# trevordblack/Physically_Based_Renderer

Measured on AMD Instinct MI355X. Metric: shaded pixels/sec (Mpix/s) + achieved HBM GB/s, 4K G-buffer, 64 lights, higher is better.
Workload: dtype f32

## Files before the change

physically_based_renderer_amd/csrc/pbr_balanced.h:

```cpp
#pragma once
#include <cstdint>
#include <type_traits>

#include "pbr_device_math.h"
#include "pbr_device_math_x2.h"
#include "shade_kernels.h"

namespace pbr {

constexpr int kBalRec = 7;

#ifndef PBR_BAL_PROFILE
#define PBR_BAL_PROFILE 0
#endif
#if PBR_BAL_PROFILE
static __device__ unsigned long long* g_bal_prof_buf;
#define BAL_PROF_T(v) const long long v = (long long)__builtin_amdgcn_s_memtime()
#define BAL_PROF_ADD(slot_, val_) do { if ((threadIdx.x & 63) == 0) bal_prof[slot_] += (unsigned long long)(val_); } while (0)
#else
#define BAL_PROF_T(v)
#define BAL_PROF_ADD(i, x)
#endif

constexpr int kBalLdsStride = kBalMaxLights + 4;
// ... 185 lines not shown
}

__device__ __forceinline__ void wave_lds_sync() {
    __builtin_amdgcn_fence(__ATOMIC_RELEASE, "wavefront");
    __builtin_amdgcn_wave_barrier();
    __builtin_amdgcn_fence(__ATOMIC_ACQUIRE, "wavefront");
}
__device__ __forceinline__ void group_lds_sync(bool block) {
    if (block) {
        asm volatile("s_waitcnt lgkmcnt(0)" ::: "memory");
        __syncthreads();
    } else {
        wave_lds_sync();
    }
}

template <bool FINITE>
__device__ __forceinline__ float bal_wave_min(float v) {
    if constexpr (FINITE) return wave_min_finite(v);
    else return wave_min_dpp(v);
}
template <bool FINITE>
__device__ __forceinline__ float bal_wave_max(float v) {
    if constexpr (FINITE) return wave_max_finite(v);
    else return wave_max_dpp(v);
}
template <bool FINITE>
__device__ __forceinline__ float bal_fmin(float a, float b) {
    if constexpr (FINITE) return fmin_finite(a, b);
    else return fminf(a, b);
}
template <bool FINITE>
__device__ __forceinline__ float bal_fmax(float a, float b) {
    if constexpr (FINITE) return fmax_finite(a, b);
    else return fmaxf(a, b);
}

__device__ __forceinline__ void push_skip_bits4(uint32_t& ma, uint32_t& mb, float4 x, float4 y, float4 z,
                                                const f3x2& n, v2 kb) {
    const v2 x01 = v2{x.x, x.y}, x23 = v2{x.z, x.w}, y01 = v2{y.x, y.y}, y23 = v2{y.z, y.w};
    const v2 z01 = v2{z.x, z.y}, z23 = v2{z.z, z.w};
    const v2 ta01 = vfma(splat(n.x.x), x01, vfma(splat(n.y.x), y01, vfma(splat(n.z.x), z01, splat(kb.x))));
    const v2 ta23 = vfma(splat(n.x.x), x23, vfma(splat(n.y.x), y23, vfma(splat(n.z.x), z23, splat(kb.x))));
    const v2 tb01 = vfma(splat(n.x.y), x01, vfma(splat(n.y.y), y01, vfma(splat(n.z.y), z01, splat(kb.y))));
    const v2 tb23 = vfma(splat(n.x.y), x23, vfma(splat(n.y.y), y23, vfma(splat(n.z.y), z23, splat(kb.y))));
    ma = __builtin_amdgcn_alignbit(ma, __float_as_uint(ta23.y), 31);
    mb = __builtin_amdgcn_alignbit(mb, __float_as_uint(tb23.y), 31);
    ma = __builtin_amdgcn_alignbit(ma, __float_as_uint(ta23.x), 31);
    mb = __builtin_amdgcn_alignbit(mb, __float_as_uint(tb23.x), 31);
    ma = __builtin_amdgcn_alignbit(ma, __float_as_uint(ta01.y), 31);
    mb = __builtin_amdgcn_alignbit(mb, __float_as_uint(tb01.y), 31);
    ma = __builtin_amdgcn_alignbit(ma, __float_as_uint(ta01.x), 31);
    mb = __builtin_amdgcn_alignbit(mb, __float_as_uint(tb01.x), 31);
}

__device__ __forceinline__ void read_pair_lights(const float* lds_lights, int j0, int j1, f3x2& lp, f3x2& ls) {
    typedef __attribute__((address_space(3))) const float lds_float;
    j0 = PBR_BOUNDS(j0, kBalMaxLights + 1, kBoundsLds);
    j1 = PBR_BOUNDS(j1, kBalMaxLights + 1, kBoundsLds);
    const uint32_t base = (uint32_t)(uintptr_t)(const lds_float*)lds_lights;
    const uint32_t a0 = base + 4u * (uint32_t)j0, a1 = base + 4u * (uint32_t)j1;
    float x0, x1, y0, y1, z0, z1, r0, r1, g0, g1, u0, u1;
    static_assert(kBalLdsStride * 4 == 272, "offsets below");
    asm volatile(
        "ds_read_b32 %0, %12\n\t"
        "ds_read_b32 %1, %13\n\t"
        "ds_read_b32 %2, %12 offset:272\n\t"
        "ds_read_b32 %3, %13 offset:272\n\t"
        "ds_read_b32 %4, %12 offset:544\n\t"
        "ds_read_b32 %5, %13 offset:544\n\t"
        "ds_read_b32 %6, %12 offset:816\n\t"
        "ds_read_b32 %7, %13 offset:816\n\t"
        "ds_read_b32 %8, %12 offset:1088\n\t"
        "ds_read_b32 %9, %13 offset:1088\n\t"
        "ds_read_b32 %10, %12 offset:1360\n\t"
        "ds_read_b32 %11, %13 offset:1360\n\t"
        "s_waitcnt lgkmcnt(0)"
        : "=&v"(x0), "=&v"(x1), "=&v"(y0), "=&v"(y1), "=&v"(z0), "=&v"(z1), "=&v"(r0), "=&v"(r1), "=&v"(g0),
          "=&v"(g1), "=&v"(u0), "=&v"(u1)
        : "v"(a0), "v"(a1)
        : "memory");
    lp = f3x2{v2{x0, x1}, v2{y0, y1}, v2{z0, z1}};
    ls = f3x2{v2{r0, r1}, v2{g0, g1}, v2{u0, u1}};
}

constexpr float kBalNearVL = 0.0625f;
static_assert(PBR_POW5_FAST3_GLIBC_FROM >= 1.0f - 0.5f * kBalNearVL + 0x1p-14f,
              "a |V + L| >= kBalNearVL item has x < 0.9688: pow5_fast3's glibc band (a build switch) must start above it");
__device__ __forceinline__ void faithful_point_items2(const ItemPixel& q, const f3x2& lp, const f3x2& ls, m2& ok,
                                                      f3x2& sum, uint64_t live) {
    f3x2 l = f3x2{lp.x - q.pos.x, lp.y - q.pos.y, lp.z - q.pos.z};
    const v2 dist = sqrt_nr(dot3(l, l));
    const Recip2 rdist = recip_nr(dist);
    l = f3x2{div_nr(l.x, rdist), div_nr(l.y, rdist), div_nr(l.z, rdist)};
    const f3x2 vl = f3x2{q.v.x + l.x, q.v.y + l.y, q.v.z + l.z};
    const v2 svl = sqrt_nr(dot3(vl, vl));
    const Recip2 rvl = recip_nr(svl);
    const f3x2 h = f3x2{div_nr(vl.x, rvl), div_nr(vl.y, rvl), div_nr(vl.z, rvl)};
    const v2 att = rdist.r * rdist.r;
    const f3x2 n = splat3(q.n.x, q.n.y, q.n.z);
    const v2 n_dot_h = dot3_sat(n, h);
    const v2 inner = ((n_dot_h * n_dot_h) * q.a2m1 + 1.0f);
    const v2 den = inner * inner;
    const v2 n_dot_l = dot3_sat(n, l);
    const v2 r = rcp_hw((den * vfma(n_dot_l, splat(q.omk), splat(q.k))) * vfma(splat(q.nv), n_dot_l, splat(0.001f)));
    const v2 x = 1.0f - dot3_sat(h, splat3(q.v.x, q.v.y, q.v.z));
// ... 6 lines not shown
        if (x.y > PBR_POW5_FAST3_GLIBC_FROM && on(live)) p.y = pow5_glibc(x.y);
    }
    const f3x2 f = f3x2{q.f0.x + q.omf0.x * p, q.f0.y + q.omf0.y * p, q.f0.z + q.omf0.z * p};
    const v2 kr = (q.a2gv * n_dot_l) * r;
    const v2 w = att * n_dot_l;
    sum.x = vfma(vfma(kr, f.x, vfma(-f.x, splat(q.mab.x), splat(q.mab.x))), ls.x * w, sum.x);
    sum.y = vfma(vfma(kr, f.y, vfma(-f.y, splat(q.mab.y), splat(q.mab.y))), ls.y * w, sum.y);
    sum.z = vfma(vfma(kr, f.z, vfma(-f.z, splat(q.mab.z), splat(q.mab.z))), ls.z * w, sum.z);
}

__device__ __forceinline__ f3x2 exact_point_items2(const ItemPixelX& p, const f3x2& lp, const f3x2& ls, m2& ok,
                                                   uint64_t live) {
    PixelInvariants2 q;
    q.n = splat3(p.n.x, p.n.y, p.n.z);
    q.v = splat3(p.v.x, p.v.y, p.v.z);
    q.albedo = splat3(p.albedo.x, p.albedo.y, p.albedo.z);
    q.f0 = splat3(p.f0.x, p.f0.y, p.f0.z);
    q.one_minus_f0 = splat3(p.omf0.x, p.omf0.y, p.omf0.z);
    q.one_minus_metal = splat(p.omm);
    q.a_sqr = splat(p.a_sqr);
    q.a_sqr_minus_1 = splat(p.a2m1);
    q.k = splat(p.k);
    q.one_minus_k = splat(p.omk);
    q.ggx_v = splat(p.ggx_v);
    q.four_n_dot_v = splat(p.nv4);
    q.f0_nonzero = m2{~0ull, ~0ull};
    f3x2 l = f3x2{lp.x - p.pos.x, lp.y - p.pos.y, lp.z - p.pos.z};
    const v2 dist = sqrt_nr(dot3(l, l));
    const Recip2 rdist = recip_nr(dist);
    l = f3x2{div_nr(l.x, rdist), div_nr(l.y, rdist), div_nr(l.z, rdist)};
    const f3x2 h = normalize_x2(add3(q.v, l), ok);
    const v2 dsat = max_dsat(dist);
    const v2 att = recip_nr(dsat * dsat).r;
    return brdf_x2<true, true>(q, f3x2{ls.x * att, ls.y * att, ls.z * att}, l, h, ok, live);
}

struct BalMasks {
    uint32_t a0, a1, c0, c1;
    bool near_a, near_b;
};

constexpr float kBalDistLoFaithful = 0.01f;
constexpr float kBalDistLoExact = 0x1p-20f;

__device__ __forceinline__ m2 beyond_range(const f3x2& pos, float lx, float ly, float lz) {
    const f3x2 l = f3x2{splat(lx) - pos.x, splat(ly) - pos.y, splat(lz) - pos.z};
    const v2 x = dot3(l, l);
    return mask2(x.x > 10000.0f, x.y > 10000.0f);
}

template <bool EXACT>
__device__ __forceinline__ BalMasks balanced_pass1(const f3x2& pos, const f3x2& n, bool live_a, bool live_b, int nl,
                                                   float dist_lo, BalancedWaveLds& w, const float* lds_lights,
                                                   unsigned long long* bal_prof = nullptr) {
    const int lane_id = (int)(threadIdx.x & 63);
    BAL_PROF_T(t0);
    const float big = 3.0e38f;
    const f3 pa = lane(pos, 0), pb = lane(pos, 1);
    constexpr bool F = !EXACT;
    const float mnx = bal_wave_min<F>(bal_fmin<F>(live_a ? pa.x : big, live_b ? pb.x : big));
    const float mny = bal_wave_min<F>(bal_fmin<F>(live_a ? pa.y : big, live_b ? pb.y : big));
    const float mnz = bal_wave_min<F>(bal_fmin<F>(live_a ? pa.z : big, live_b ? pb.z : big));
    const float mxx = bal_wave_max<F>(bal_fmax<F>(live_a ? pa.x : -big, live_b ? pb.x : -big));
    const float mxy = bal_wave_max<F>(bal_fmax<F>(live_a ? pa.y : -big, live_b ? pb.y : -big));
    const float mxz = bal_wave_max<F>(bal_fmax<F>(live_a ? pa.z : -big, live_b ? pb.z : -big));
    const float cx = 0.5f * mnx + 0.5f * mxx, cy = 0.5f * mny + 0.5f * mxy, cz = 0.5f * mnz + 0.5f * mxz;
    const float r = (0.5f * (mxx - mnx) + 0.5f * (mxy - mny)) + 0.5f * (mxz - mnz);
    const float slack = r + (fabsf(cx) + fabsf(cy) + fabsf(cz)) * 0x1p-22f;
    const float pmax = bal_wave_max<F>(bal_fmax<F>(live_a ? (fabsf(pa.x) + fabsf(pa.y)) + fabsf(pa.z) : 0.0f,
                                                   live_b ? (fabsf(pb.x) + fabsf(pb.y)) + fabsf(pb.z) : 0.0f));
    float bj = 0.0f;
    bool near = true, far = false;
    bool close = false;
    if (lane_id < nl) {
        const float lx = lds_lights[lane_id], ly = lds_lights[kBalLdsStride + lane_id],
                    lz = lds_lights[2 * kBalLdsStride + lane_id];
        const float b0 = ((fabsf(lx - cx) + fabsf(ly - cy)) + fabsf(lz - cz)) + slack;
        const float fr = ((fabsf(lx) + fabsf(ly)) + fabsf(lz)) + pmax;
        bj = (b0 + 0.125f * fr) * (1.0f + 0x1p-20f);
        const float fx = fmaxf(fabsf(lx - mnx), fabsf(lx - mxx)), fy = fmaxf(fabsf(ly - mny), fabsf(ly - mxy)),
                    fz = fmaxf(fabsf(lz - mnz), fabsf(lz - mxz));
        const float gx = fmaxf(fmaxf(mnx - lx, lx - mxx), 0.0f), gy = fmaxf(fmaxf(mny - ly, ly - mxy), 0.0f),
                    gz = fmaxf(fmaxf(mnz - lz, lz - mxz), 0.0f);
        near = (fx * fx + fy * fy) + fz * fz <= 99.9f * 99.9f;
        far = (gx * gx + gy * gy) + gz * gz >= 100.1f * 100.1f;
        close = !((gx * gx + gy * gy) + gz * gz >= (1.02f * dist_lo) * (1.02f * dist_lo));
    }
    const float bmax = bal_wave_max<F>(bj);
    const uint64_t far_m = lanes(far), cross_m = lanes(!near && !far), close_m = lanes(close);
    const v2 cn = v2{0x1p-18f * ((fabsf(n.x.x) + fabsf(n.y.x)) + fabsf(n.z.x)),
                     0x1p-18f * ((fabsf(n.x.y) + fabsf(n.y.y)) + fabsf(n.z.y))};
    const v2 nd = -vfma(n.z, pos.z, vfma(n.y, pos.y, n.x * pos.x));
    const v2 kb = vfma(cn, splat(bmax), nd);
    uint32_t a0 = 0, a1 = 0, c0 = 0, c1 = 0;
    typedef __attribute__((address_space(3))) const float lds_float;
    const uint32_t lbase = (uint32_t)(uintptr_t)(const lds_float*)lds_lights;
    auto word = [&](int qbase, uint32_t& ma, uint32_t& mb) {
        for (int k = 6; k >= 0; k -= 2) {
            const uint32_t la = lbase + 16u * (uint32_t)(qbase + k);
            float4 x1, y1, z1, x0, y0, z0;
            asm volatile(
                "ds_read_b128 %0, %6 offset:16\n\t"
                "ds_read_b128 %1, %6 offset:288\n\t"
                "ds_read_b128 %2, %6 offset:560\n\t"
                "ds_read_b128 %3, %6\n\t"
                "ds_read_b128 %4, %6 offset:272\n\t"
                "ds_read_b128 %5, %6 offset:544\n\t"
                "s_waitcnt lgkmcnt(0)"
                : "=&v"(x1), "=&v"(y1), "=&v"(z1), "=&v"(x0), "=&v"(y0), "=&v"(z0)
                : "v"(la)
                : "memory");
            push_skip_bits4(ma, mb, x1, y1, z1, n, kb);
            push_skip_bits4(ma, mb, x0, y0, z0, n, kb);
        }
    };
    const int n0 = nl < 32 ? nl : 32;
    if (nl > 32) word(8, a1, c1);
    word(0, a0, c0);
    const int n1 = nl - n0;
    const uint32_t k0 = (n0 == 32 ? ~0u : (1u << n0) - 1u) & ~(uint32_t)far_m,
                   k1 = (n1 == 32 ? ~0u : (1u << n1) - 1u) & ~(uint32_t)(far_m >> 32);
    a0 = live_a ? ~a0 & k0 : 0u;
    c0 = live_b ? ~c0 & k0 : 0u;
    a1 = live_a ? ~a1 & k1 : 0u;
    c1 = live_b ? ~c1 & k1 : 0u;
    for (uint64_t cm = cross_m; cm != 0; cm &= cm - 1) {
        const int j = __builtin_ctzll(cm);
        const m2 out = beyond_range(pos, lds_lights[j], lds_lights[kBalLdsStride + j], lds_lights[2 * kBalLdsStride + j]);
        const uint32_t bit = 1u << (j & 31);
        const uint32_t oa = on(out.x) ? bit : 0u, ob = on(out.y) ? bit : 0u;
        if (j < 32) {
            a0 &= ~oa;
            c0 &= ~ob;
        } else {
            a1 &= ~oa;
            c1 &= ~ob;
        }
    }
    bool near_a = false, near_b = false;
    for (uint64_t cm = close_m; cm != 0; cm &= cm - 1) {
        const int j = __builtin_ctzll(cm);
        const f3x2 l = f3x2{splat(lds_lights[j]) - pos.x, splat(lds_lights[kBalLdsStride + j]) - pos.y,
                            splat(lds_lights[2 * kBalLdsStride + j]) - pos.z};
        const m2 ok = ge(sqrt_nr(dot3(l, l)), dist_lo);
        const uint32_t bit = 1u << (j & 31);
        near_a = near_a || (((j < 32 ? a0 : a1) & bit) != 0 && !on(ok.x));
        near_b = near_b || (((j < 32 ? c0 : c1) & bit) != 0 && !on(ok.y));
    }

    BAL_PROF_T(t1);
    BAL_PROF_ADD(0, t1 - t0);
    return BalMasks{a0, a1, c0, c1, near_a, near_b};
}

__device__ __forceinline__ int wave_live_items(const BalMasks& bm) {
    return wave_sum_dpp((__popc(bm.a0) + __popc(bm.a1)) + (__popc(bm.c0) + __popc(bm.c1)));
}


template <bool EXACT>
__device__ __forceinline__ void lighting_balanced_points(const PixelInvariants2& q, const Faithful2& fi,
                                                         const f3x2& pos, bool live_a, bool live_b, BalMasks bm,
                                                         BalancedWaveLds& w, const float* lds_lights, f3x2& sum,
                                                         m2& redo, unsigned long long* bal_prof = nullptr) {
    const int lane_id = (int)(threadIdx.x & 63);
    const uint32_t a0 = bm.a0, a1 = bm.a1, c0 = bm.c0, c1 = bm.c1;
    redo |= mask2(bm.near_a, bm.near_b);
    constexpr int R = EXACT ? kBalRecX : kBalRec;
    BAL_PROF_T(t1);
    PBR_PHASE("rank");

// ... 154 lines not shown
```

physically_based_renderer_amd/csrc/pbr_census.h:

```cpp
#pragma once

#ifndef PBR_CENSUS
#define PBR_CENSUS 0
#endif
#if PBR_CENSUS
#define PBR_PHASE(name)                          \
    do {                                         \
        __builtin_amdgcn_sched_barrier(0);       \
        asm volatile("; @phase " name);          \
        __builtin_amdgcn_sched_barrier(0);       \
    } while (0)
#else
#define PBR_PHASE(name) \
    do {                \
    } while (0)
#endif
#define PBR_COLD(name) PBR_PHASE("cold_" name)
```

physically_based_renderer_amd/csrc/pbr_context.hip:

```cpp
#include <cmath>
#include <cstdlib>
#include <cstring>
#include <new>

#include "pbr_context_impl.h"
#include "pbr_debug_bounds.h"
#include "pbr_build_info.h"

extern "C" {
extern const char pbr_unit_info_shade_kernels[] __attribute__((weak));
extern const char pbr_unit_info_shade_kernels_bal[] __attribute__((weak));
extern const char pbr_unit_info_frontend_kernels[] __attribute__((weak));
extern const char pbr_unit_info_pbr_frontend[] __attribute__((weak));
extern const char pbr_unit_info_gbuffer_fill[] __attribute__((weak));
__attribute__((used)) const char pbr_unit_info_pbr_context[] =
    PBR_UNIT_INFO("pbr_context", PBR_BI_SWITCH(PBR_DEBUG_BOUNDS));
}

namespace {

constexpr float kQuarterStrengthLo = 0x1p-34f, kQuarterStrengthHi = 0x1p50f;

constexpr float kFaithfulStrengthLo = 0x1p-25f, kFaithfulStrengthHi = 0x1p50f;

// ... 139 lines not shown
    return PBR_OK;
}

extern "C" {

int pbr_abi_version(void) { return PBR_ABI_VERSION; }

const char* pbr_build_info(void) {
    static const std::string info = [] {
        std::string r = "{\"abi\": " + std::to_string(PBR_ABI_VERSION) + ", \"units\": [";
        bool first = true;
        for (const char* u : {pbr_unit_info_pbr_context, pbr_unit_info_pbr_frontend, pbr_unit_info_shade_kernels,
                              pbr_unit_info_shade_kernels_bal, pbr_unit_info_frontend_kernels,
                              pbr_unit_info_gbuffer_fill}) {
            if (u == nullptr) continue;
            r += first ? "" : ", ";
            r += u;
            first = false;
        }
        return r + "]}";
    }();
    return info.c_str();
}

const char* pbr_strerror(int status) {
    switch (status) {
        case PBR_OK: return "ok";
        case PBR_ERR_INVALID_ARGUMENT: return "invalid argument";
        case PBR_ERR_NO_DEVICE: return "no HIP device";
        case PBR_ERR_OUT_OF_MEMORY: return "out of device memory";
        case PBR_ERR_LAUNCH: return "kernel launch failed";
        case PBR_ERR_HIP: return "HIP runtime error";
        case PBR_ERR_NOT_READY: return "pass or environment map not set";
        case PBR_ERR_UNSUPPORTED: return "unsupported";
        default: return "unknown status";
    }
}

const char* pbr_last_error(const pbr_context* ctx) { return ctx ? ctx->last_error.c_str() : ""; }

int pbr_context_create(int device, pbr_context** out_ctx) {
    if (!out_ctx) return PBR_ERR_INVALID_ARGUMENT;
    *out_ctx = nullptr;
    int count = 0;
    if (hipGetDeviceCount(&count) != hipSuccess || count <= 0) return PBR_ERR_NO_DEVICE;
    if (device < 0 || device >= count) return PBR_ERR_INVALID_ARGUMENT;
    pbr_context* ctx = new (std::nothrow) pbr_context();
    if (!ctx) return PBR_ERR_OUT_OF_MEMORY;
    ctx->device = device;
    if (const char* e = std::getenv("PBR_PIXELS_PER_THREAD")) ctx->pixels_per_thread = std::atoi(e) == 1 ? 1 : 2;
    if (const char* e = std::getenv("PBR_BALANCED_MIN")) ctx->balanced_min = std::atoi(e);
    if (const char* e = std::getenv("PBR_LEAN")) ctx->lean = std::atoi(e) != 0;
    if (const char* e = std::getenv("PBR_RANK_PER_WAVE")) ctx->rank_per_wave = std::atoi(e) != 0;
    DeviceGuard g(device);
    if (!g.ok) {
        delete ctx;
        return PBR_ERR_NO_DEVICE;
    }
    hipError_t e = arm_bounds(device);
    for (int i = 0; e == hipSuccess && i < pbr_context::kSlots; ++i) {
        e = hipHostMalloc(reinterpret_cast<void**>(&ctx->slots[i].h), sizeof(pbr_light) * PBR_MAX_LIGHTS,
                          hipHostMallocDefault);
        if (e == hipSuccess) e = hipEventCreateWithFlags(&ctx->slots[i].copied, hipEventDisableTiming);
    }
    if (e != hipSuccess) {
        pbr_context_destroy(ctx);
        return e == hipErrorOutOfMemory ? PBR_ERR_OUT_OF_MEMORY : PBR_ERR_HIP;
    }
    *out_ctx = ctx;
    return PBR_OK;
}

int pbr_context_destroy(pbr_context* ctx) {
    if (!ctx) return PBR_ERR_INVALID_ARGUMENT;
    {
        DeviceGuard g(ctx->device);
        (void)hipDeviceSynchronize();
        for (Resource* r : ctx->resources) {
            for (void** m : r->mem)
                if (m && *m) (void)hipFreeAsync(*m, nullptr);
            if (r->written) (void)hipEventDestroy(r->written);
        }
        for (pbr_context::LightSlot& sl : ctx->slots) {
            if (sl.copied) (void)hipEventDestroy(sl.copied);
            if (sl.h) (void)hipHostFree(sl.h);
        }
        for (StreamState& st : ctx->streams) release_stream_state(st);
        (void)hipDeviceSynchronize();
    }
    delete ctx;
    return PBR_OK;
}

int pbr_set_pass(pbr_context* ctx, const pbr_pass_desc* pass, void* stream) {
    if (!ctx || !pass) return PBR_ERR_INVALID_ARGUMENT;
    const int nd = pass->num_dir_lights, np = pass->num_point_lights, ns = pass->num_spot_lights;
    if (nd < 0 || np < 0 || ns < 0) return PBR_ERR_INVALID_ARGUMENT;
    const long long n = (long long)nd + np + ns;
    if (n > PBR_MAX_LIGHTS) return PBR_ERR_INVALID_ARGUMENT;
    if (n > 0 && !pass->lights) return PBR_ERR_INVALID_ARGUMENT;
    if (!is_ambient_mode(pass->ambient_mode)) return PBR_ERR_INVALID_ARGUMENT;
    const uint32_t known =
        PBR_FLAG_F0_PLANE | PBR_FLAG_APPLY_AO | PBR_FLAG_TILED_CULLING | PBR_FLAG_EXACT_ONLY | PBR_FLAG_FAITHFUL |
        PBR_FLAG_ALPHA_TEST;
    if (pass->flags & ~known) return PBR_ERR_INVALID_ARGUMENT;

// ... 146 lines not shown
    const bool alpha_test = (ctx->flags & PBR_FLAG_ALPHA_TEST) != 0;
    if (alpha_test && !gb->opacity) return PBR_ERR_INVALID_ARGUMENT;
    if (ctx->ambient_mode == PBR_AMBIENT_IBL_DIFFUSE && !ctx->env.d) return PBR_ERR_NOT_READY;
    if (fr->coverage && !ctx->sky.d) return PBR_ERR_NOT_READY;

    pbr::LaunchArgs a{};
    const float* planes[15] = {gb->pos_w[0], gb->pos_w[1], gb->pos_w[2], gb->normal_w[0], gb->normal_w[1],
                               gb->normal_w[2], gb->albedo[0], gb->albedo[1], gb->albedo[2], gb->metallic,
                               gb->roughness, gb->ao, gb->f0[0], gb->f0[1], gb->f0[2]};
    for (int i = 0; i < 15; ++i) a.gb.plane[i] = planes[i] ? planes[i] : planes[0];
    a.gb.plane[15] = alpha_test ? gb->opacity : planes[0];
    a.gb.alpha_test = alpha_test;
    a.gb.width = gb->width;
    a.gb.height = gb->height;
    a.gb.row_stride = gb->row_stride;
    a.gb.pairs_aligned = (gb->row_stride % 2) == 0;
    for (int i = 0; i < 16; ++i)
        if (!aligned(a.gb.plane[i], 8)) a.gb.pairs_aligned = false;
    a.ps = ctx->pass;
    a.ps.env_w = ctx->env.w;
    a.ps.env_h = ctx->env.h;
    a.ps.sky_w = ctx->sky.w;
    a.ps.sky_h = ctx->sky.h;
    a.lights = ctx->cur_slot >= 0 ? ctx->slots[ctx->cur_slot].d : nullptr;
    a.env = ctx->env.d;
    a.frame.out = fr->out;
    a.frame.out_stride = fr->out_row_stride;
    a.frame.format = fr->format == PBR_OUTPUT_RGBA8_UNORM ? pbr::kOutRgba8 : pbr::kOutRgba32f;
    a.frame.coverage = fr->coverage;
    a.frame.coverage_stride = fr->coverage_row_stride;
    a.frame.sky = ctx->sky.d;
    a.frame.width = gb->width - (debug_bounds_skew() ? 1 : 0);
    a.frame.height = gb->height;
    a.ambient_mode = ctx->ambient_mode;
    a.f0_plane = f0_plane;
    a.apply_ao = apply_ao;
    a.cull = cull;
    a.exact_only = (ctx->flags & PBR_FLAG_EXACT_ONLY) != 0;
    a.ps.faithful = (ctx->flags & PBR_FLAG_FAITHFUL) && !a.exact_only && ctx->faithful_pass_ok &&
                    (ctx->ambient_mode != PBR_AMBIENT_IBL_DIFFUSE || ctx->env.faithful_ok);
    if (a.ps.faithful && ctx->faithful_count_terms) a.ps.faithful = 2;
    a.pixels_per_thread = ctx->pixels_per_thread;
    constexpr int kBalancedMinFaithful = 22, kBalancedMinExact = 18;
    const int bal_min = ctx->balanced_min >= 0 ? ctx->balanced_min
                        : a.ps.faithful == 1   ? kBalancedMinFaithful
                                               : kBalancedMinExact;
    const bool bal_ok = !cull && a.pixels_per_thread == 2 && bal_min > 0 && ctx->points_flag_ok &&
                        a.ps.n_spot == 0 && a.ps.n_point >= bal_min && a.ps.n_point <= pbr::kBalMaxLights;
    a.ps.balanced = !bal_ok                                                ? 0
                    : a.ps.faithful == 1                                   ? 1
                    : a.ps.faithful == 0 && !a.exact_only && a.ps.n_dir == 0 && ctx->points_quarter_ok ? 2
                                                                           : 0;
    if (a.ps.balanced != 0 && ctx->rank_per_wave) a.ps.balanced |= pbr::kBalRankPerWave;

    if (const int rc = en.open(stream, "shade stream")) return rc;
    const hipStream_t s = en.s;
    const int si = en.si;
    hipError_t e = hipSuccess;
    StreamState& st = ctx->streams[si];
    {
        const int64_t tiles = pbr::shade_tile_count(gb->width, gb->height, a.pixels_per_thread);
        const int64_t slots = tiles * pbr::shade_stat_slots_per_tile(a.pixels_per_thread);
        if (slots > st.stats_capacity) {
            if (st.d_stats) {
                e = hipStreamSynchronize(s);
                if (e != hipSuccess) return fail_hip(ctx, e, "pass stats sync");
                (void)hipFree(st.d_stats);
                st.d_stats = nullptr;
                st.stats_capacity = 0;
            }
            e = hipMalloc(&st.d_stats, pbr::kStatsPerBlock * sizeof(int32_t) * (size_t)slots);
            if (e != hipSuccess) return fail_hip(ctx, e, "pass stats hipMalloc");
            st.stats_capacity = slots;
        }
        st.tiles = tiles;
        st.slots = slots;
        st.culled = cull;
        a.tile_kept = st.d_stats;
        a.lean = ctx->lean && a.pixels_per_thread == 2 && a.ps.balanced == 0 && !fr->coverage && !a.exact_only;
    }
    const bool reads_lights = ctx->cur_slot >= 0 && a.ps.n_dir + a.ps.n_point + a.ps.n_spot > 0;
    if (reads_lights) e = before_read(ctx->slots[ctx->cur_slot].use, s, si);
    if (e == hipSuccess && ctx->ambient_mode == PBR_AMBIENT_IBL_DIFFUSE) e = before_read(ctx->env.use, s, si);
    if (e == hipSuccess && fr->coverage) e = before_read(ctx->sky.use, s, si);
    if (e != hipSuccess) return fail_hip(ctx, e, "shade order");
    e = pbr::launch_shade(a, s);
    if (e != hipSuccess) return fail_hip(ctx, e, "shade_tile_kernel launch", PBR_ERR_LAUNCH);
    st.kernel = pbr::launched_kernel(a);
    if (const int rc = after_launch(ctx, si, s, "shade record")) return rc;
    ctx->last_stream = si;
    return PBR_OK;
}

}

extern "C" {

int pbr_set_env_map(pbr_context* ctx, const uint16_t* texels, int32_t width, int32_t height, void* stream) {
    return ctx ? set_texture(ctx, ctx->env, texels, true, width, height, stream, "pbr_set_env_map")
               : PBR_ERR_INVALID_ARGUMENT;
}

int pbr_set_env_map_f32(pbr_context* ctx, const float* texels, int32_t width, int32_t height, void* stream) {
    return ctx ? set_texture(ctx, ctx->env, texels, false, width, height, stream, "pbr_set_env_map_f32")
               : PBR_ERR_INVALID_ARGUMENT;
}
// ... 117 lines not shown
```

physically_based_renderer_amd/csrc/pbr_context_impl.h:

```cpp
#pragma once
#include <hip/hip_runtime.h>

#include <cstdint>
#include <mutex>
#include <optional>
#include <string>
#include <vector>

#include "pbr/pbr_shade.h"
#include "shade_kernels.h"
#include "frontend_kernels.h"

#pragma GCC visibility push(hidden)

struct StreamState {
    hipStream_t stream = nullptr;
    hipEvent_t last_pass = nullptr;
    int32_t* d_stats = nullptr;
    int64_t stats_capacity = 0;
    int64_t tiles = 0, slots = 0;
    bool culled = false;
    std::string kernel;
    struct Raster {
        char* d = nullptr;
// ... 44 lines not shown
        float4* d = nullptr;
        int w = 0, h = 0, capacity = 0;
        bool faithful_ok = true;
        Resource use;
        explicit Texture(std::vector<Resource*>& l) : use(l, &d_u16, &d) {}
    };
    Texture env{resources}, sky{resources};
    struct Materials {
        pbr::MaterialRec* d_table = nullptr;
        uint32_t* d_texels = nullptr;
        int n = 0;
        int64_t n_texels = 0;
        std::vector<uint32_t> flags;
        std::vector<pbr::MaterialTex> place;
        std::vector<int32_t> slot_tex;
        bool set = false;
        Resource use;
        explicit Materials(std::vector<Resource*>& l) : use(l, &d_table, &d_texels) {}
    };
    Materials mats{resources};
    struct Mips {
        char* d_tables = nullptr;
        uint32_t* d_texels = nullptr;
        const pbr::MipSlot* d_slots = nullptr;
        const pbr::MaterialTex* d_levels = nullptr;
        int64_t n_levels = 0, n_texels = 0;
        bool set = false;
        Resource use;
        explicit Mips(std::vector<Resource*>& l) : use(l, &d_tables, &d_texels) {}
    };
    Mips mips{resources};
    struct MeshPlace {
        uint32_t vtx_base, n_vertices, idx_base, n_indices;
    };
    struct Meshes {
        float* d_vertices = nullptr;
        uint32_t* d_indices = nullptr;
        int64_t n_vertices = 0, n_indices = 0;
        std::vector<MeshPlace> place;
        bool set = false;
        Resource use;
        explicit Meshes(std::vector<Resource*>& l) : use(l, &d_vertices, &d_indices) {}
    };
    Meshes meshes{resources};
    pbr::PassArgs pass{};
    int ambient_mode = 0;
    uint32_t flags = 0;
    bool pass_set = false;
    bool faithful_pass_ok = false;
    bool faithful_count_terms = false;
    int last_stream = -1;
    int balanced_min = -1;
    bool rank_per_wave = false;
    bool points_flag_ok = false;
    bool points_quarter_ok = false;
    int pixels_per_thread = 2;
    bool lean = true;
    std::string last_error;
    std::mutex mu;
};

struct DeviceGuard {
    int prev = -1;
    bool ok = false;
    explicit DeviceGuard(int dev) {
        if (hipGetDevice(&prev) != hipSuccess) prev = -1;
        ok = hipSetDevice(dev) == hipSuccess;
    }
    ~DeviceGuard() {
        if (prev >= 0) (void)hipSetDevice(prev);
    }
};

int fail_hip(pbr_context* ctx, hipError_t e, const char* what, int status = PBR_ERR_HIP);
int stream_index(pbr_context* ctx, hipStream_t s, hipError_t& e);
hipError_t before_write(pbr_context* ctx, Resource& r, hipStream_t w, int wi);
hipError_t free_after_readers(pbr_context* ctx, Resource& r, void* p, hipStream_t w, int wi);
hipError_t after_write(Resource& r, hipStream_t w, int wi);
hipError_t before_read(Resource& r, hipStream_t s, int si);
int after_launch(pbr_context* ctx, int si, hipStream_t s, const char* what);
bool debug_bounds_skew();

inline bool aligned(const void* p, uintptr_t a) { return (reinterpret_cast<uintptr_t>(p) & (a - 1)) == 0; }

template <class T>
bool planes_ok(T* const* p, int n, uintptr_t min_align, bool& vec) {
    for (int i = 0; i < n; ++i) {
        if (!p[i] || !aligned(p[i], min_align)) return false;
        vec = vec && aligned(p[i], 8);
    }
    return true;
}

struct Entry {
    pbr_context* ctx;
    std::lock_guard<std::mutex> lk;
    std::optional<DeviceGuard> g;
    hipStream_t s = nullptr;
    int si = -1;
    explicit Entry(pbr_context* c) : ctx(c), lk(c->mu) {}
    int device(void* stream) {
        g.emplace(ctx->device);
        s = static_cast<hipStream_t>(stream);
        return g->ok ? PBR_OK : PBR_ERR_NO_DEVICE;
    }
    int open(void* stream, const char* what) {
// ... 31 lines not shown
```

physically_based_renderer_amd/csrc/shade_kernels.h:

```cpp
#pragma once
#include <hip/hip_runtime.h>

#include <cstdint>
#include <string>

#include "pbr_census.h"

namespace pbr {

constexpr int kAmbientConstant = 0;
constexpr int kAmbientIblDiffuse = 1;

struct GBufferArgs {
    const float* plane[16];
    int width, height;
    int64_t row_stride;
    bool pairs_aligned;
    bool alpha_test;
};

struct PassArgs {
    float eye[3];
    float ambient[3];
    float fresnel_r0[3];
    float opacity;
    int n_dir, n_point, n_spot;
    int env_w, env_h;
    int sky_w, sky_h;
    int eye_ok;
    int balanced;
    int faithful;
};

constexpr int kBalKindMask = 3;
constexpr int kBalRankPerWave = 4;

constexpr int kOutRgba32f = 0;
constexpr int kOutRgba8 = 1;

struct FrameArgs {
    void* out;
    int64_t out_stride;
    int format;
    const uint8_t* coverage;
    int64_t coverage_stride;
    const float4* sky;
    int width, height;
};

enum StatField {
    kStatCullKept = 0,
    kStatCullTiles = 1,
    kStatExactPixels = 2,
    kStatLightTerms = 3,
    kStatGeometryPixels = 4,
    kStatBackfaceTests = 5,
    kStatsPerBlock = 6
};
constexpr int kBalMaxLights = 64;

struct LaunchArgs {
    GBufferArgs gb;
    PassArgs ps;
    const float4* lights;
    const float4* env;
    FrameArgs frame;
    int32_t* tile_kept;
    int ambient_mode;
    bool f0_plane, apply_ao, cull;
    bool exact_only;
    int pixels_per_thread;
    bool lean;
};

hipError_t launch_shade(const LaunchArgs& a, hipStream_t stream);
std::string launched_kernel(const LaunchArgs& a);
int64_t shade_tile_count(int width, int height, int pixels_per_thread);
int shade_stat_slots_per_tile(int pixels_per_thread);
hipError_t debug_bal_profile(unsigned long long* out8, bool reset);
hipError_t debug_wave_timeline(unsigned long long* buf, long long cap);
hipError_t debug_bounds_publish(uint32_t* buf);
hipError_t launch_decode_unorm16(const uint16_t* src, float4* dst, int n_texels, hipStream_t stream);

}
```

physically_based_renderer_amd/csrc/shade_tile_kernel.h:

```cpp
#pragma once
#include <hip/hip_runtime.h>

#include <cstdint>

#include "shade_common.h"
#include "shade_wave_timeline.h"
#include "shade_light_loops.h"
#include "shade_pixel.h"

namespace pbr {

template <int AMBIENT, bool F0_PLANE, bool APPLY_AO, bool CULL, int BAL = 0>
__global__ __launch_bounds__(kBlock, PBR_X2_MIN_WAVES) void shade_tile_kernel(
    GBufferArgs gb, PassArgs ps, const float4* __restrict__ lights, const float4* __restrict__ env, FrameArgs fr,
    int32_t* __restrict__ tile_kept, bool exact_only) {
    __shared__ Lds s;
    TL_BEGIN();
    PBR_PHASE("entry");
#if PBR_BAL_PROFILE
    const long long t_entry = (long long)__builtin_amdgcn_s_memtime();
    unsigned long long* bal_prof = s.prof[__builtin_amdgcn_readfirstlane(threadIdx.x) >> 6];
    if ((threadIdx.x & 63) < 16) bal_prof[threadIdx.x & 63] = 0;
#endif
    load_libm_tables<AMBIENT == kAmbientIblDiffuse, kBlock>();
// ... 37 lines not shown
        const bool finite = (!ga || (isfinite(pa.x) && isfinite(pa.y) && isfinite(pa.z))) &&
                            (!gb_ || (isfinite(pb.x) && isfinite(pb.y) && isfinite(pb.z)));
        const float big = 3.0e38f;
        wb.mn[0] = uniform_f(wave_min(fminf(ga ? pa.x : big, gb_ ? pb.x : big)));
        wb.mn[1] = uniform_f(wave_min(fminf(ga ? pa.y : big, gb_ ? pb.y : big)));
        wb.mn[2] = uniform_f(wave_min(fminf(ga ? pa.z : big, gb_ ? pb.z : big)));
        wb.mx[0] = uniform_f(wave_max(fmaxf(ga ? pa.x : -big, gb_ ? pb.x : -big)));
        wb.mx[1] = uniform_f(wave_max(fmaxf(ga ? pa.y : -big, gb_ ? pb.y : -big)));
        wb.mx[2] = uniform_f(wave_max(fmaxf(ga ? pa.z : -big, gb_ ? pb.z : -big)));
        cull_enabled = lanes(!finite) == 0;
    }

    int kept_total = 0;
    int bal_items = -1;
    m2 redo = m2{0, 0};
    f3x2 pos2 = p.pos;
    f3x2 d2 = splat3(0.0f, 0.0f, 0.0f);
    bool faithful_wave = false;
    TL_RT(3);
    auto vote = [&](bool yes) {
        if ((tid & 63) == 0) s.bal[wslot].vote = yes;
    };
    auto vote_no = [&]() {
        if constexpr (BAL != 0) {
            vote(false);
            __syncthreads();
        }
    };
    if (wave_geometry) {
        const v2 nn = dot3(p.n, p.n);
        const bool lean_lane = ok_a && ok_b && nn.x <= 1.0f + 0x1p-20f && nn.y <= 1.0f + 0x1p-20f &&
                               f0_nonzero(lane(p.f0, 0)) && f0_nonzero(lane(p.f0, 1));
        const bool faithful_lane =
            ps.faithful && ok_a && ok_b && p.albedo.x.x >= 0.0f && p.albedo.y.x >= 0.0f && p.albedo.z.x >= 0.0f &&
            p.albedo.x.y >= 0.0f && p.albedo.y.y >= 0.0f && p.albedo.z.y >= 0.0f && p.f0.x.x <= 1.0f &&
            p.f0.y.x <= 1.0f && p.f0.z.x <= 1.0f && p.f0.x.y <= 1.0f && p.f0.y.y <= 1.0f && p.f0.z.y <= 1.0f &&
            p.f0.x.x >= 0.0f && p.f0.y.x >= 0.0f && p.f0.z.x >= 0.0f && p.f0.x.y >= 0.0f && p.f0.y.y >= 0.0f &&
            p.f0.z.y >= 0.0f;
        faithful_wave = BAL != 2 && ps.faithful && lanes(!faithful_lane) == 0;
        if (CULL && faithful_wave && ps.faithful == 2)
            faithful_wave = wave_light_terms(lights, ps, wb, cull_enabled) <= kFaithfulMaxTerms;
        const bool lean_wave = lanes(!lean_lane) == 0;
        if (faithful_wave && lean_wave) {
            if constexpr (BAL == 1 && !CULL) {
#if PBR_BAL_PROFILE
                BAL_PROF_ADD(7, (long long)__builtin_amdgcn_s_memtime() - t_entry);
                unsigned long long* prof = s.prof[wslot];
#else
                unsigned long long* prof = nullptr;
#endif
                PBR_PHASE("pass1");
                vote(!(ps.balanced & kBalRankPerWave));
                const BalMasks bm = balanced_pass1<false>(p.pos, p.n, ga, gb_, ps.n_point, kBalDistLoFaithful, s.bal[wslot],
                                                   s.bal_light, prof);
                bal_items = wave_live_items(bm);
                PBR_PHASE("invariants");
                launder(p);
                q2 = pair_invariants(p, ps, fast2);
                faithful_scale(q2);
                d2 = lighting_fast<false, true, true, true>(q2, p.pos, fast2, lights, ps, wb, cull_enabled, redo,
                                                            kept_total, &s.bal[wslot], s.bal_light, ga, gb_, bm,
                                                            prof);
#if PBR_BAL_PROFILE
                const long long t_l1 = (long long)__builtin_amdgcn_s_memtime();
#endif
                PBR_PHASE("invariants2");
                launder(p);
                q2 = pair_finish_invariants(p, ps, fast2);
                pos2 = p.pos;
#if PBR_BAL_PROFILE
                const v2 dep = dot3(q2.n, q2.v);
                if (dep.x == 12345.0f) pos2.x.x = 0.5f;
                BAL_PROF_ADD(8, (long long)__builtin_amdgcn_s_memtime() - t_l1);
#endif
            } else {
                vote_no();
                form_q2();
                if (!CULL) faithful_scale(q2);
#if PBR_BAL_PROFILE
                const long long t_u0 = (long long)__builtin_amdgcn_s_memtime();
                BAL_PROF_ADD(11, t_u0 - t_entry);
                BAL_PROF_ADD(13, 1);
#endif
                d2 = lighting_fast<CULL, true, true>(q2, pos2, fast2, lights, ps, wb, cull_enabled, redo, kept_total);
                if (!CULL) faithful_unscale(q2);
#if PBR_BAL_PROFILE
                const v2 dep = d2.x + d2.y;
                if (dep.x == 12345.0f) pos2.x.x = 0.5f;
                BAL_PROF_ADD(12, (long long)__builtin_amdgcn_s_memtime() - t_u0);
#endif
            }
        } else if (faithful_wave) {
            PBR_COLD("faithful_nonlean");
            vote_no();
            form_q2();
            if (!CULL) faithful_scale(q2);
            d2 = lighting_fast<CULL, false, true>(q2, pos2, fast2, lights, ps, wb, cull_enabled, redo, kept_total);
            if (!CULL) faithful_unscale(q2);
        } else if (lean_wave) {
            PBR_PHASE("xpass1");
            if constexpr (BAL == 2 && !CULL) {
#if PBR_BAL_PROFILE
                unsigned long long* prof = s.prof[wslot];
#else
                unsigned long long* prof = nullptr;
#endif
                auto reload = [&]() {
                    asm volatile("" ::: "memory");
                    const int rl = lane_id_fresh();
                    const int rx = blockIdx.x * kTileW + 2 * (rl & 31);
                    const int ry = tile_y * kTileH + 2 * wave_id + (rl >> 5);
                    const int64_t rrow = (int64_t)ry * gb.row_stride + rx;
                    p = load_pair<F0_PLANE, APPLY_AO>(gb, ps, va ? rrow : 0, vb ? rrow + 1 : 0,
                                                      vb && gb.pairs_aligned);
                };
                vote(!(ps.balanced & kBalRankPerWave));
                const BalMasks bm = balanced_pass1<true>(p.pos, p.n, ga, gb_, ps.n_point, kBalDistLoExact, s.bal[wslot],
                                                   s.bal_light, prof);
                bal_items = wave_live_items(bm);
                PBR_PHASE("xinvariants");
                q2 = pair_invariants(p, ps, fast2);
                d2 = lighting_fast<false, true, false, true>(q2, p.pos, fast2, lights, ps, wb, cull_enabled, redo,
                                                             kept_total, &s.bal[wslot], s.bal_light, ga, gb_, bm,
                                                             prof);
                PBR_PHASE("xinvariants2");
                reload();
                q2 = pair_invariants(p, ps, fast2);
                pos2 = p.pos;
            } else {
                vote_no();
                form_q2();
                d2 = lighting_fast<CULL, true>(q2, pos2, fast2, lights, ps, wb, cull_enabled, redo, kept_total);
            }
        } else {
            PBR_COLD("general");
            vote_no();
            form_q2();
            d2 = lighting_fast<CULL, false>(q2, pos2, fast2, lights, ps, wb, cull_enabled, redo, kept_total);
        }
    } else {
        PBR_COLD("background");
        vote_no();
        form_q2();
    }
    TL_RT(4);
    const PixelInvariants ua = unpack_invariants(q2, 0), ub = unpack_invariants(q2, 1);
    f3 da = lane(d2, 0), db = lane(d2, 1);
    const bool need_a = ga && on(redo.x), need_b = gb_ && on(redo.y);
    PBR_PHASE("stats_repass");
    const int n_exact = __popcll(lanes(need_a)) + __popcll(lanes(need_b));
    const int geo_px = __popcll(lanes(ga)) + __popcll(lanes(gb_));
    if ((tid & 63) == 0 && tile_kept != nullptr) {
        const int64_t slot = ((int64_t)tile_y * gridDim.x + blockIdx.x) * (kBlock / 64) + wave_id;
        const int n_ps = CULL ? kept_total : ps.n_point + ps.n_spot;
        const int terms = !wave_geometry ? 0 : bal_items >= 0 ? bal_items + ps.n_dir * geo_px : (ps.n_dir + n_ps) * geo_px;
        int32_t* st = tile_kept + kStatsPerBlock * slot;
        st[kStatCullKept] = CULL && wave_geometry ? kept_total : 0;
        st[kStatCullTiles] = CULL && wave_geometry ? 1 : 0;
        st[kStatExactPixels] = n_exact;
        st[kStatLightTerms] = terms;
        st[kStatGeometryPixels] = geo_px;
        st[kStatBackfaceTests] = wave_geometry && bal_items >= 0 ? ps.n_point * geo_px : 0;
    }
#if PBR_BAL_PROFILE
    const long long t_b0 = (long long)__builtin_amdgcn_s_memtime();
#endif
    if (BAL == 0 && n_exact != 0) {
        PBR_COLD("exact_repass");
        f3 ea, eb;
        lighting_exact_wave(ua, ub, lane(pos2, 0), lane(pos2, 1), need_a, need_b, lights, ps, ea, eb);
        if (need_a) da = ea;
// ... 54 lines not shown
```

Measured before the change: 10750.

## Compute pass1 light-skip plane tests with f32 MFMA outer products instead of VALU

```diff
diff --git a/physically_based_renderer_amd/csrc/pbr_balanced.h b/physically_based_renderer_amd/csrc/pbr_balanced.h
--- a/physically_based_renderer_amd/csrc/pbr_balanced.h
+++ b/physically_based_renderer_amd/csrc/pbr_balanced.h
@@ -261,6 +261,28 @@
     mb = __builtin_amdgcn_alignbit(mb, __float_as_uint(tb01.y), 31);
     ma = __builtin_amdgcn_alignbit(ma, __float_as_uint(ta01.x), 31);
     mb = __builtin_amdgcn_alignbit(mb, __float_as_uint(tb01.x), 31);
+}
+
+typedef float bal_acc32 __attribute__((ext_vector_type(32)));
+
+__device__ __forceinline__ int bal_mfma_light(int lane_id) {
+    return 16 * ((lane_id >> 2) & 1) + 4 * ((lane_id & 31) >> 3) + (lane_id & 3);
+}
+
+__device__ __forceinline__ uint32_t skip_word_mfma(float lx, float ly, float lz, float nx, float ny, float nz, float kb,
+                                                   int xlane, uint32_t sel) {
+    bal_acc32 acc;
+#pragma unroll
+    for (int i = 0; i < 32; ++i) acc[i] = 0.0f;
+    acc = __builtin_amdgcn_mfma_f32_32x32x1f32(1.0f, kb, acc, 0, 0, 0);
+    acc = __builtin_amdgcn_mfma_f32_32x32x1f32(lz, nz, acc, 0, 0, 0);
+    acc = __builtin_amdgcn_mfma_f32_32x32x1f32(ly, ny, acc, 0, 0, 0);
+    acc = __builtin_amdgcn_mfma_f32_32x32x1f32(lx, nx, acc, 0, 0, 0);
+    uint32_t m = 0;
+#pragma unroll
+    for (int i = 31; i >= 0; --i) m = __builtin_amdgcn_alignbit(m, __float_as_uint(acc[i]), 31);
+    const uint32_t partner = (uint32_t)__builtin_amdgcn_ds_bpermute(xlane, (int)m);
+    return __builtin_amdgcn_perm(m, partner, sel);
 }
 
 __device__ __forceinline__ void read_pair_lights(const float* lds_lights, int j0, int j1, f3x2& lp, f3x2& ls) {
@@ -373,7 +395,7 @@
 template <bool EXACT>
 __device__ __forceinline__ BalMasks balanced_pass1(const f3x2& pos, const f3x2& n, bool live_a, bool live_b, int nl,
                                                    float dist_lo, BalancedWaveLds& w, const float* lds_lights,
-                                                   unsigned long long* bal_prof = nullptr) {
+                                                   bool valu, unsigned long long* bal_prof = nullptr) {
     const int lane_id = (int)(threadIdx.x & 63);
     BAL_PROF_T(t0);
     const float big = 3.0e38f;
@@ -418,6 +440,7 @@
     const uint32_t lbase = (uint32_t)(uintptr_t)(const lds_float*)lds_lights;
     auto word = [&](int qbase, uint32_t& ma, uint32_t& mb) {
         for (int k = 6; k >= 0; k -= 2) {
+            PBR_TAKEN("pass1_valu_word");
             const uint32_t la = lbase + 16u * (uint32_t)(qbase + k);
             float4 x1, y1, z1, x0, y0, z0;
             asm volatile(
@@ -436,8 +459,26 @@
         }
     };
     const int n0 = nl < 32 ? nl : 32;
-    if (nl > 32) word(8, a1, c1);
-    word(0, a0, c0);
+    if (__builtin_expect(valu, 0)) {
+        PBR_COLD("pass1_valu");
+        if (nl > 32) word(8, a1, c1);
+        word(0, a0, c0);
+    } else {
+        const int lj = PBR_BOUNDS(bal_mfma_light(lane_id), 32, kBoundsLds);
+        const int xlane = 4 * (lane_id ^ 32);
+        const uint32_t sel = lane_id < 32 ? 0x01000504u : 0x07060302u;
+        const float x0 = lds_lights[lj], y0 = lds_lights[kBalLdsStride + lj], z0 = lds_lights[2 * kBalLdsStride + lj];
+        if (nl > 32) {
+            PBR_TAKEN("pass1_word1");
+            const float x1 = lds_lights[32 + lj], y1 = lds_lights[kBalLdsStride + 32 + lj],
+                        z1 = lds_lights[2 * kBalLdsStride + 32 + lj];
+            a1 = skip_word_mfma(x1, y1, z1, n.x.x, n.y.x, n.z.x, kb.x, xlane, sel);
+            c1 = skip_word_mfma(x1, y1, z1, n.x.y, n.y.y, n.z.y, kb.y, xlane, sel);
+        }
+        PBR_TAKEN("pass1_word0");
+        a0 = skip_word_mfma(x0, y0, z0, n.x.x, n.y.x, n.z.x, kb.x, xlane, sel);
+        c0 = skip_word_mfma(x0, y0, z0, n.x.y, n.y.y, n.z.y, kb.y, xlane, sel);
+    }
     const int n1 = nl - n0;
     const uint32_t k0 = (n0 == 32 ? ~0u : (1u << n0) - 1u) & ~(uint32_t)far_m,
                    k1 = (n1 == 32 ? ~0u : (1u << n1) - 1u) & ~(uint32_t)(far_m >> 32);
diff --git a/physically_based_renderer_amd/csrc/pbr_census.h b/physically_based_renderer_amd/csrc/pbr_census.h
--- a/physically_based_renderer_amd/csrc/pbr_census.h
+++ b/physically_based_renderer_amd/csrc/pbr_census.h
@@ -15,4 +15,16 @@
     do {                \
     } while (0)
 #endif
+#if PBR_CENSUS
+#define PBR_TAKEN(name)                          \
+    do {                                         \
+        __builtin_amdgcn_sched_barrier(0);       \
+        asm volatile("; @taken " name);          \
+        __builtin_amdgcn_sched_barrier(0);       \
+    } while (0)
+#else
+#define PBR_TAKEN(name) \
+    do {                \
+    } while (0)
+#endif
 #define PBR_COLD(name) PBR_PHASE("cold_" name)
diff --git a/physically_based_renderer_amd/csrc/pbr_context.hip b/physically_based_renderer_amd/csrc/pbr_context.hip
--- a/physically_based_renderer_amd/csrc/pbr_context.hip
+++ b/physically_based_renderer_amd/csrc/pbr_context.hip
@@ -215,6 +215,7 @@
     if (const char* e = std::getenv("PBR_BALANCED_MIN")) ctx->balanced_min = std::atoi(e);
     if (const char* e = std::getenv("PBR_LEAN")) ctx->lean = std::atoi(e) != 0;
     if (const char* e = std::getenv("PBR_RANK_PER_WAVE")) ctx->rank_per_wave = std::atoi(e) != 0;
+    if (const char* e = std::getenv("PBR_PASS1_VALU")) ctx->pass1_valu = std::atoi(e) != 0;
     DeviceGuard g(device);
     if (!g.ok) {
         delete ctx;
@@ -467,6 +468,7 @@
                     : a.ps.faithful == 0 && !a.exact_only && a.ps.n_dir == 0 && ctx->points_quarter_ok ? 2
                                                                            : 0;
     if (a.ps.balanced != 0 && ctx->rank_per_wave) a.ps.balanced |= pbr::kBalRankPerWave;
+    if (a.ps.balanced != 0 && ctx->pass1_valu) a.ps.balanced |= pbr::kBalPass1Valu;
 
     if (const int rc = en.open(stream, "shade stream")) return rc;
     const hipStream_t s = en.s;
diff --git a/physically_based_renderer_amd/csrc/pbr_context_impl.h b/physically_based_renderer_amd/csrc/pbr_context_impl.h
--- a/physically_based_renderer_amd/csrc/pbr_context_impl.h
+++ b/physically_based_renderer_amd/csrc/pbr_context_impl.h
@@ -120,6 +120,7 @@
     int last_stream = -1;
     int balanced_min = -1;
     bool rank_per_wave = false;
+    bool pass1_valu = false;
     bool points_flag_ok = false;
     bool points_quarter_ok = false;
     int pixels_per_thread = 2;
diff --git a/physically_based_renderer_amd/csrc/shade_kernels.h b/physically_based_renderer_amd/csrc/shade_kernels.h
--- a/physically_based_renderer_amd/csrc/shade_kernels.h
+++ b/physically_based_renderer_amd/csrc/shade_kernels.h
@@ -34,6 +34,7 @@
 
 constexpr int kBalKindMask = 3;
 constexpr int kBalRankPerWave = 4;
+constexpr int kBalPass1Valu = 8;
 
 constexpr int kOutRgba32f = 0;
 constexpr int kOutRgba8 = 1;
diff --git a/physically_based_renderer_amd/csrc/shade_tile_kernel.h b/physically_based_renderer_amd/csrc/shade_tile_kernel.h
--- a/physically_based_renderer_amd/csrc/shade_tile_kernel.h
+++ b/physically_based_renderer_amd/csrc/shade_tile_kernel.h
@@ -113,7 +113,7 @@
                 PBR_PHASE("pass1");
                 vote(!(ps.balanced & kBalRankPerWave));
                 const BalMasks bm = balanced_pass1<false>(p.pos, p.n, ga, gb_, ps.n_point, kBalDistLoFaithful, s.bal[wslot],
-                                                   s.bal_light, prof);
+                                                   s.bal_light, (ps.balanced & kBalPass1Valu) != 0, prof);
                 bal_items = wave_live_items(bm);
                 PBR_PHASE("invariants");
                 launder(p);
@@ -177,7 +177,7 @@
                 };
                 vote(!(ps.balanced & kBalRankPerWave));
                 const BalMasks bm = balanced_pass1<true>(p.pos, p.n, ga, gb_, ps.n_point, kBalDistLoExact, s.bal[wslot],
-                                                   s.bal_light, prof);
+                                                   s.bal_light, (ps.balanced & kBalPass1Valu) != 0, prof);
                 bal_items = wave_live_items(bm);
                 PBR_PHASE("xinvariants");
                 q2 = pair_invariants(p, ps, fast2);
```

After: 10830 (median of 6 runs). Within noise of the previous version (+0.7%).
